# nv-dvl/nerfmatch

Measured on AMD Instinct MI355X. Metric: rays*samples/sec, higher is better.
Workload: dtype fp16x3 (fp16 MFMA on hi/lo-split fp32 operands, three products per fp32 product, fp32 accumulate; fp32 everywhere else)

## Files before the change

nerfmatch_amd/csrc/nerf_fwd_bf16.hip:

```cpp
#include "nerf_split_chain.h"

namespace {
using namespace nmbf;

template <int PART>
__device__ __forceinline__ void tap_prefetch(Ctx& cx) {
  if constexpr (PART == 0) __builtin_amdgcn_s_barrier();
  const char* src = reinterpret_cast<const char*>(cx.tapw);
#pragma unroll
  for (int q = (PART == 0 ? 0 : 4); q < (PART == 0 ? 4 : 7); ++q) {
    const char* sp = src + q * 4096;
    const float* dp = q < 4 ? cx.tap_ring + q * 1024 : cx.tap_ipe + (q - 4) * 1024;
    const unsigned lds = (unsigned)__builtin_amdgcn_readfirstlane((int)(unsigned)(size_t)(const __attribute__((address_space(3))) float*)dp);
    unsigned m0_saved;
    asm volatile("s_mov_b32 %0, m0\n\ts_mov_b32 m0, %1\n\tglobal_load_lds_dwordx4 %2, off\n\tglobal_load_lds_dwordx4 %2, off offset:1024\n\t"
                 "global_load_lds_dwordx4 %2, off offset:2048\n\tglobal_load_lds_dwordx4 %2, off offset:3072\n\ts_mov_b32 m0, %0"
                 : "=&s"(m0_saved) : "s"(lds), "v"(sp) : "memory");
  }
}

__device__ __forceinline__ void dpp_pairs8(float (&o)[8], const float (&x)[8], const float (&y)[8], bool eight) {
  if (eight)
    asm("s_nop 1\n"
        "v_add_f32_dpp %0, %8, %8 row_mirror row_mask:0xf bank_mask:0x3\n\tv_add_f32_dpp %1, %9, %9 row_mirror row_mask:0xf bank_mask:0x3\n\t"
        "v_add_f32_dpp %2, %10, %10 row_mirror row_mask:0xf bank_mask:0x3\n\tv_add_f32_dpp %3, %11, %11 row_mirror row_mask:0xf bank_mask:0x3\n\t"
        "v_add_f32_dpp %4, %12, %12 row_mirror row_mask:0xf bank_mask:0x3\n\tv_add_f32_dpp %5, %13, %13 row_mirror row_mask:0xf bank_mask:0x3\n\t"
        "v_add_f32_dpp %6, %14, %14 row_mirror row_mask:0xf bank_mask:0x3\n\tv_add_f32_dpp %7, %15, %15 row_mirror row_mask:0xf bank_mask:0x3\n\t"
        "v_add_f32_dpp %0, %16, %16 row_mirror row_mask:0xf bank_mask:0xc\n\tv_add_f32_dpp %1, %17, %17 row_mirror row_mask:0xf bank_mask:0xc\n\t"
        "v_add_f32_dpp %2, %18, %18 row_mirror row_mask:0xf bank_mask:0xc\n\tv_add_f32_dpp %3, %19, %19 row_mirror row_mask:0xf bank_mask:0xc\n\t"
        "v_add_f32_dpp %4, %20, %20 row_mirror row_mask:0xf bank_mask:0xc\n\tv_add_f32_dpp %5, %21, %21 row_mirror row_mask:0xf bank_mask:0xc\n\t"
        "v_add_f32_dpp %6, %22, %22 row_mirror row_mask:0xf bank_mask:0xc\n\tv_add_f32_dpp %7, %23, %23 row_mirror row_mask:0xf bank_mask:0xc"
        : "=&v"(o[0]), "=&v"(o[1]), "=&v"(o[2]), "=&v"(o[3]), "=&v"(o[4]), "=&v"(o[5]), "=&v"(o[6]), "=&v"(o[7])
        : "v"(x[0]), "v"(x[1]), "v"(x[2]), "v"(x[3]), "v"(x[4]), "v"(x[5]), "v"(x[6]), "v"(x[7]),
          "v"(y[0]), "v"(y[1]), "v"(y[2]), "v"(y[3]), "v"(y[4]), "v"(y[5]), "v"(y[6]), "v"(y[7]));
  else
    asm("s_nop 1\n"
        "v_add_f32_dpp %0, %8, %8 row_half_mirror row_mask:0xf bank_mask:0x5\n\tv_add_f32_dpp %1, %9, %9 row_half_mirror row_mask:0xf bank_mask:0x5\n\t"
        "v_add_f32_dpp %2, %10, %10 row_half_mirror row_mask:0xf bank_mask:0x5\n\tv_add_f32_dpp %3, %11, %11 row_half_mirror row_mask:0xf bank_mask:0x5\n\t"
        "v_add_f32_dpp %4, %12, %12 row_half_mirror row_mask:0xf bank_mask:0x5\n\tv_add_f32_dpp %5, %13, %13 row_half_mirror row_mask:0xf bank_mask:0x5\n\t"
        "v_add_f32_dpp %6, %14, %14 row_half_mirror row_mask:0xf bank_mask:0x5\n\tv_add_f32_dpp %7, %15, %15 row_half_mirror row_mask:0xf bank_mask:0x5\n\t"
        "v_add_f32_dpp %0, %16, %16 row_half_mirror row_mask:0xf bank_mask:0xa\n\tv_add_f32_dpp %1, %17, %17 row_half_mirror row_mask:0xf bank_mask:0xa\n\t"
        "v_add_f32_dpp %2, %18, %18 row_half_mirror row_mask:0xf bank_mask:0xa\n\tv_add_f32_dpp %3, %19, %19 row_half_mirror row_mask:0xf bank_mask:0xa\n\t"
        "v_add_f32_dpp %4, %20, %20 row_half_mirror row_mask:0xf bank_mask:0xa\n\tv_add_f32_dpp %5, %21, %21 row_half_mirror row_mask:0xf bank_mask:0xa\n\t"
        "v_add_f32_dpp %6, %22, %22 row_half_mirror row_mask:0xf bank_mask:0xa\n\tv_add_f32_dpp %7, %23, %23 row_half_mirror row_mask:0xf bank_mask:0xa"
        : "=&v"(o[0]), "=&v"(o[1]), "=&v"(o[2]), "=&v"(o[3]), "=&v"(o[4]), "=&v"(o[5]), "=&v"(o[6]), "=&v"(o[7])
        : "v"(x[0]), "v"(x[1]), "v"(x[2]), "v"(x[3]), "v"(x[4]), "v"(x[5]), "v"(x[6]), "v"(x[7]),
          "v"(y[0]), "v"(y[1]), "v"(y[2]), "v"(y[3]), "v"(y[4]), "v"(y[5]), "v"(y[6]), "v"(y[7]));
}
template <int XOR>
__device__ __forceinline__ void quad_add8(float (&v)[8]) {
  if (XOR == 1)
    asm("s_nop 1\n"
        "v_add_f32_dpp %0, %0, %0 quad_perm:[1,0,3,2] row_mask:0xf bank_mask:0xf\n\tv_add_f32_dpp %1, %1, %1 quad_perm:[1,0,3,2] row_mask:0xf bank_mask:0xf\n\t"
        "v_add_f32_dpp %2, %2, %2 quad_perm:[1,0,3,2] row_mask:0xf bank_mask:0xf\n\tv_add_f32_dpp %3, %3, %3 quad_perm:[1,0,3,2] row_mask:0xf bank_mask:0xf\n\t"
        "v_add_f32_dpp %4, %4, %4 quad_perm:[1,0,3,2] row_mask:0xf bank_mask:0xf\n\tv_add_f32_dpp %5, %5, %5 quad_perm:[1,0,3,2] row_mask:0xf bank_mask:0xf\n\t"
        "v_add_f32_dpp %6, %6, %6 quad_perm:[1,0,3,2] row_mask:0xf bank_mask:0xf\n\tv_add_f32_dpp %7, %7, %7 quad_perm:[1,0,3,2] row_mask:0xf bank_mask:0xf"
        : "+v"(v[0]), "+v"(v[1]), "+v"(v[2]), "+v"(v[3]), "+v"(v[4]), "+v"(v[5]), "+v"(v[6]), "+v"(v[7]));
  else
    asm("s_nop 1\n"
        "v_add_f32_dpp %0, %0, %0 quad_perm:[2,3,0,1] row_mask:0xf bank_mask:0xf\n\tv_add_f32_dpp %1, %1, %1 quad_perm:[2,3,0,1] row_mask:0xf bank_mask:0xf\n\t"
        "v_add_f32_dpp %2, %2, %2 quad_perm:[2,3,0,1] row_mask:0xf bank_mask:0xf\n\tv_add_f32_dpp %3, %3, %3 quad_perm:[2,3,0,1] row_mask:0xf bank_mask:0xf\n\t"
        "v_add_f32_dpp %4, %4, %4 quad_perm:[2,3,0,1] row_mask:0xf bank_mask:0xf\n\tv_add_f32_dpp %5, %5, %5 quad_perm:[2,3,0,1] row_mask:0xf bank_mask:0xf\n\t"
        "v_add_f32_dpp %6, %6, %6 quad_perm:[2,3,0,1] row_mask:0xf bank_mask:0xf\n\tv_add_f32_dpp %7, %7, %7 quad_perm:[2,3,0,1] row_mask:0xf bank_mask:0xf"
        : "+v"(v[0]), "+v"(v[1]), "+v"(v[2]), "+v"(v[3]), "+v"(v[4]), "+v"(v[5]), "+v"(v[6]), "+v"(v[7]));
}
__device__ __forceinline__ f32x4 reduce_scatter_32rows(float (&v)[128], int lane) {
  float s1[64];
#pragma unroll
  for (int i = 0; i < 64; ++i) {
    const auto r = __builtin_amdgcn_permlane16_swap(__float_as_uint(v[i]), __float_as_uint(v[64 + i]), false, false);
    s1[i] = __uint_as_float(r[0]) + __uint_as_float(r[1]);
  }
  float s2[32];
#pragma unroll
  for (int b = 0; b < 4; ++b) {
    float o[8], x[8], y[8];
#pragma unroll
    for (int i = 0; i < 8; ++i) { x[i] = s1[8 * b + i]; y[i] = s1[32 + 8 * b + i]; }
    dpp_pairs8(o, x, y, true);
#pragma unroll
    for (int i = 0; i < 8; ++i) s2[8 * b + i] = o[i];
  }
  float s3[16];
#pragma unroll
  for (int b = 0; b < 2; ++b) {
    float o[8], x[8], y[8];
#pragma unroll
    for (int i = 0; i < 8; ++i) { x[i] = s2[8 * b + i]; y[i] = s2[16 + 8 * b + i]; }
    dpp_pairs8(o, x, y, false);
#pragma unroll
    for (int i = 0; i < 8; ++i) s3[8 * b + i] = o[i];
  }
  float lo8[8], hi8[8];
#pragma unroll
  for (int i = 0; i < 8; ++i) { lo8[i] = s3[i]; hi8[i] = s3[8 + i]; }
  quad_add8<2>(lo8); quad_add8<2>(hi8);
  float s4[8];
#pragma unroll
  for (int i = 0; i < 8; ++i) s4[i] = (lane & 2) ? hi8[i] : lo8[i];
  float t8[8] = {s4[0], s4[1], s4[2], s4[3], s4[4], s4[5], s4[6], s4[7]};
  quad_add8<1>(t8);
  return (lane & 1) ? f32x4{t8[4], t8[5], t8[6], t8[7]} : f32x4{t8[0], t8[1], t8[2], t8[3]};
}

#define NM_MLP_DONE_WAIT() __builtin_amdgcn_s_waitcnt(0x0070)
#define NM_EPI_BARRIER() asm volatile("s_waitcnt lgkmcnt(0)\n\ts_barrier" ::: "memory")
template <int P>
__device__ __forceinline__ void nerf_fwd_body(const NerfArgs& a) {
  __shared__ __attribute__((aligned(16))) float sm[LDS_TOTAL];
  float* const sm_small = sm + LDS_SMALL;
  float* const ring = sm + LDS_RING;
  float* const sm_ipe = sm + LDS_IPE;
  float* const sm_sigma = sm + LDS_SCR;
  float* const sm_rgb = sm_sigma + TILE;
  float* const sm_t0 = sm_rgb + 3 * TILE;
  float* const sm_t1 = sm_t0 + TILE;
  float* const sm_mean = sm_t1 + TILE;
  float* const sm_dn = sm_mean + 3 * TILE;
  float* const sm_w = sm_dn + TILE;
  float* const sm_misc = sm_w + TILE;
  float* const sm_feat = sm + LDS_FEAT;
  float* const sm_part = sm_feat;
  float* const sm_ex = sm + LDS_EX;
  int* const sm_lray = reinterpret_cast<int*>(sm + LDS_LEFT);
  float* const sm_lT = sm + LDS_LEFT + TILE;
  unsigned* const sm_rng = reinterpret_cast<unsigned*>(sm + LDS_RNG);

  const int tid = threadIdx.x, lane = tid & 63, wave = tid >> 6, s = lane & 31, hi = lane >> 5;
  const bool tail_ok = a.left && !(a.tail_viol && *a.tail_viol != 0);
  const int S = a.S, R = a.R;
  const int Sa = tail_ok ? a.Sa : S;
  const int left = tail_ok ? 1 : 0;
  const int ntiles = tail_ok ? a.ntiles : a.ntiles_full;
  const int SP = Sa < TILE ? Sa : TILE;
  const int nr = TILE / SP;
  const int nchunks = (Sa + TILE - 1) / TILE;
  const bool need_rgb = !(a.flags & NM_NERF_SKIP_RGB);
  const bool feat_max = (a.flags & NM_NERF_FEAT_MAX) != 0;
  const bool need_tap = (a.feat != nullptr) || (a.sfeat != nullptr);
  const int tap = (a.tap < 0 || a.tap > 7) ? 7 : a.tap;
  const int nslots = need_rgb ? NSLOT_FULL : NSLOT_NORGB;
  const char* const blob_slots = a.blob + (size_t)SMALL_PAD * 4;

  for (int i = tid; i < SMALL / 4; i += 256) reinterpret_cast<f32x4*>(sm_small)[i] = reinterpret_cast<const f32x4*>(a.blob)[i];
  if constexpr (P == 2) {
#pragma unroll
    for (int k = 0; k < NRANGE; ++k) sm_rng[k * 256 + tid] = 0u;
  }

  int nleft = 0;
  int bid = blockIdx.x;
#pragma unroll 1
  for (;;) {
  bool lo_pass = false;
  if (left && (nleft > TILE - 4 || (bid >= ntiles && nleft > 0))) lo_pass = true;
  else if (bid >= ntiles) break;
  const int nent = lo_pass ? nleft : 0;
  TRACE(0);
  if (need_rgb && !lo_pass && tid < nr * 48) {
    const int r2 = tid / 48, f = tid % 48;
    const int ray2 = bid * nr + r2;
    const float* rq = a.rays + (size_t)(ray2 < R ? ray2 : R - 1) * 12 + 8;
    float v = 0.f;
    if (f < 24) {
      const int k = (f % 12) / 3;
      const float xe = rq[f % 3] * (float)(1 << k);
      v = nm_sinf(f < 12 ? xe : xe + 1.57079637050628662109375f);
    } else if (f < 27) {
      v = rq[f - 24];
    } else if (f < 43) {
      v = a.app_row ? a.app_row[f - 27] : 0.f;
    }
    if constexpr (P == 2) {
      v *= reinterpret_cast<const float*>(a.blob)[OFF_INSCALE + (f < 27 ? 1 : 2)];
      __hip_atomic_fetch_max(sm_rng + 9 * 256 + tid, __float_as_uint(fabsf(v)), __ATOMIC_RELAXED, __HIP_MEMORY_SCOPE_WORKGROUP);
    }
    sm_ex[tid] = v;
  }
  __syncthreads();
  TRACE(1);

  const int js = wave * 32 + s;
  const int rl = js / SP;
  const int ray = lo_pass ? (js < nent ? sm_lray[js] : R) : bid * nr + rl;
  const int rc = lo_pass ? sm_lray[js < nent ? js : 0] : (ray < R ? ray : R - 1);
  const float* rp = a.rays + (size_t)rc * 12;
  const float o0 = rp[0], o1 = rp[1], o2 = rp[2], d0 = rp[3], d1 = rp[4], d2 = rp[5], radius = rp[11];
  const float dsq0 = d0 * d0, dsq1 = d1 * d1, dsq2 = d2 * d2;
  const float dmag = fmaxf(1e-10f, (dsq0 + dsq1) + dsq2);
  const float dnorm = sqrtf((dsq0 + dsq1) + dsq2);
  const float nul0 = 1.0f - dsq0 / dmag, nul1 = 1.0f - dsq1 / dmag, nul2 = 1.0f - dsq2 / dmag;

  float red_acc = 0.f;
  float carryT = 1.f;
  float best_w = -1.f;
  float feat_run = 0.f;

  const int nch = lo_pass ? 1 : nchunks;
  for (int chunk = 0; chunk < nch; ++chunk) {
    const int sidx = lo_pass ? Sa : chunk * TILE + (js % SP);
    const float t0 = a.t[(size_t)rc * (S + 1) + sidx];
    const float t1 = a.t[(size_t)rc * (S + 1) + sidx + 1];
    const float mu = (t0 + t1) / 2.0f, hw = (t1 - t0) / 2.0f;
    const float mu2 = mu * mu, hw2 = hw * hw, hw4 = hw2 * hw2;
    const float denom = fmaxf(1.1920928955078125e-07f, 3.0f * mu2 + hw2);
    const float t_mean = mu + (2.0f * mu * hw2) / denom;
    const float t_var = hw2 / 3.0f - (float)(4.0 / 15.0) * ((hw4 * (12.0f * mu2 - hw2)) / (denom * denom));
    const float r_var = (radius * radius) * ((mu2 / 4.0f + (float)(5.0 / 12.0) * hw2) - (float)(4.0 / 15.0) * hw4 / denom);
    float mean[3] = {d0 * t_mean + o0, d1 * t_mean + o1, d2 * t_mean + o2};
    float var[3] = {t_var * dsq0 + r_var * nul0, t_var * dsq1 + r_var * nul1, t_var * dsq2 + r_var * nul2};
    if (a.var_scale > 0.f) {
      var[0] *= a.var_scale; var[1] *= a.var_scale; var[2] *= a.var_scale;
    }
    if (hi == 0) {
      sm_t0[js] = t0; sm_t1[js] = t1;
      sm_mean[js] = mean[0]; sm_mean[TILE + js] = mean[1]; sm_mean[2 * TILE + js] = mean[2];
      sm_dn[js] = dnorm;
    }

#pragma unroll
    for (int g0 = 0; g0 < ring_ahead<P>(); ++g0) dma_slot<P>(blob_slots, g0, ring, wave, lane);

    {
      float* dst = sm_ipe + wave * (XS * 2 * 64 * 4) + lane * 4;
      const float ipe_scale = sm_small[OFF_INSCALE];
      const float phl = hi ? 1.57079637050628662109375f : 0.f;
#pragma unroll
      for (int m = 0; m < XS; ++m) {
        float v8[8];
#pragma unroll
        for (int i = 0; i < 8; ++i) {
          const int idx = 8 * m + i;
          const bool live = idx < 45;
          const int ax = (live ? idx : 0) % 3, sb = (live ? idx : 0) / 3;
          const float mu = mean[ax], vr = var[ax];
          const float sc = (float)(1 << sb);
          const float xe = mu * sc;
          float v = __builtin_amdgcn_exp2f((-0.5f * (vr * (sc * sc))) * 1.44269504088896340736f) * sin32(xe + phl);
          if constexpr (P == 2) v *= ipe_scale;
          v8[i] = live ? v : 0.f;
        }
        if constexpr (is_split<P>()) {
          bf16x8 h8, l8;
          split8_p<P>(v8, h8, l8);
          *reinterpret_cast<u32x4*>(dst + (m * 2 + 0) * 256) = __builtin_bit_cast(u32x4, h8);
          *reinterpret_cast<u32x4*>(dst + (m * 2 + 1) * 256) = __builtin_bit_cast(u32x4, l8);
        } else {
          *reinterpret_cast<u32x4*>(dst + m * 256) = __builtin_bit_cast(u32x4, pack8_f16(v8));
        }
      }
    }

    TRACE(2);
    Ctx cx;
    cx.blob_slots = blob_slots; cx.ring = ring; cx.sm_small = sm_small;
    cx.tapw = reinterpret_cast<f32x4*>(a.ws) + ((size_t)blockIdx.x * 4 + wave) * 32 * 64 + lane;
    cx.nslots = nslots; cx.wave = wave; cx.lane = lane; cx.hi = hi; cx.tap = need_tap ? tap : -1; cx.g = 0; cx.sig_part = 0.f;
    cx.vmax = 0.f; cx.rng = sm_rng + tid; cx.sc = 1.f;
    cx.tap_pref = need_tap && !lo_pass; cx.rgb = need_rgb;
    cx.tap_ring = ring + wave * SLOT_FLOATS; cx.tap_ipe = sm_ipe + wave * (XS * 2 * 64 * 4);
    if constexpr (is_split<P>()) {
      NM_WAIT_VMCNT(8);
      __builtin_amdgcn_s_barrier();
    } else {
      ring_acquire<P>(blob_slots, 0, nslots, ring, wave, lane);
    }
    load_half<P>(cx.opA, ring, lane, 0);
    if constexpr (P == 1) load_half<1>(cx.opB, ring, lane, 1);
    const float* ipe_src = sm_ipe + wave * (XS * 2 * 64 * 4) + lane * 4;
    f32x16 acc[8];
    ipe_steps<P, true>(acc, cx, ipe_src);
    finish_layer<P>(acc, 0, cx);
    TRACE(3);
#pragma unroll 1
    for (int l = 1; l < 8; ++l) {
      layer_pass<P>(acc, l, cx, ipe_src);
      TRACE(3 + l);
    }
    float c_r = 0.f, c_g = 0.f, c_b = 0.f;
    if (!need_rgb) {
      if (cx.tap == 7) dump_tap(7, cx);
      NM_MLP_DONE_WAIT();
      if (cx.tap_pref) tap_prefetch<0>(cx);
      alpha_head(cx);
      if (cx.tap_pref) tap_prefetch<1>(cx);
    } else {
      const int hh = launder(lane) >> 5;
      const float* exr = sm_ex + launder(rl) * 48 + 8 * hh;
      f32x16 av[4];
      views_hidden<P>(av, cx);
      fold_range<P>(cx, 7);
      bf16x8 exh[VS], exl[VS];
#pragma unroll
      for (int e = 0; e < VS; ++e) {
        float v8[8];
        if (!lo_pass) {
          const f32x4 e0 = *reinterpret_cast<const f32x4*>(exr + 16 * e), e1 = *reinterpret_cast<const f32x4*>(exr + 16 * e + 4);
          v8[0] = e0[0]; v8[1] = e0[1]; v8[2] = e0[2]; v8[3] = e0[3]; v8[4] = e1[0]; v8[5] = e1[1]; v8[6] = e1[2]; v8[7] = e1[3];
        } else {
          const float* rq = a.rays + (size_t)launder(rc) * 12 + 8;
          const float vd0 = rq[0], vd1 = rq[1], vd2 = rq[2];
#pragma unroll
          for (int i = 0; i < 8; ++i) {
            const int f = 16 * e + 8 * hh + i;
            const int ax = f % 3;
            const float dax = ax == 0 ? vd0 : ax == 1 ? vd1 : vd2;
            float v = 0.f;
            if (f < 24) {
              const float xe = dax * (float)(1 << ((f % 12) / 3));
              v = nm_sinf(f < 12 ? xe : xe + 1.57079637050628662109375f);
            } else if (f < 27) {
              v = dax;
            } else if (f < 43) {
              v = a.app_row ? a.app_row[f - 27] : 0.f;
            }
            if constexpr (P == 2) v *= sm_small[OFF_INSCALE + (f < 27 ? 1 : 2)];
            v8[i] = v;
          }
        }
        if constexpr (is_split<P>()) split8_p<P>(v8, exh[e], exl[e]);
        else exh[e] = exl[e] = pack8_f16(v8);
      }
      views_extras<P>(av, cx, exh, exl);
      TRACE(11);
      NM_MLP_DONE_WAIT();
      if (cx.tap_pref) tap_prefetch<0>(cx);
      const float* bv = sm_small + OFF_BVIEWS + 4 * hh;
      const float* wr = sm_small + OFF_WRGB + 4 * hh;
      float pr = 0.f, pg = 0.f, pb = 0.f;
#pragma unroll
      for (int ob = 0; ob < 4; ++ob) {
#pragma unroll
        for (int q = 0; q < 4; ++q) {
          const f32x4 b4 = *reinterpret_cast<const f32x4*>(bv + ob * 32 + 8 * q);
          const f32x4 wr4 = *reinterpret_cast<const f32x4*>(wr + ob * 32 + 8 * q);
          const f32x4 wg4 = *reinterpret_cast<const f32x4*>(wr + 128 + ob * 32 + 8 * q);
          const f32x4 wb4 = *reinterpret_cast<const f32x4*>(wr + 256 + ob * 32 + 8 * q);
#pragma unroll
          for (int e = 0; e < 4; ++e) {
            const float hv = __builtin_fmaxf(acc_read(av[ob][4 * q + e]) + b4[e], 0.f);
            pr = NM_FMA(hv, wr4[e], pr);
            pg = NM_FMA(hv, wg4[e], pg);
            pb = NM_FMA(hv, wb4[e], pb);
          }
        }
      }
      pr = (pr + nm_shfl_xor32(pr)) + sm_small[OFF_MISC + 1];
      pg = (pg + nm_shfl_xor32(pg)) + sm_small[OFF_MISC + 2];
      pb = (pb + nm_shfl_xor32(pb)) + sm_small[OFF_MISC + 3];
      c_r = 1.0f / (1.0f + expf(-pr));
      c_g = 1.0f / (1.0f + expf(-pg));
      c_b = 1.0f / (1.0f + expf(-pb));
      if (cx.tap_pref) tap_prefetch<1>(cx);
    }
    const float sigma_raw = (cx.sig_part + nm_shfl_xor32(cx.sig_part)) + sm_small[OFF_MISC];
    TRACE(12);
    {
      const int jsw = launder(js);
      if ((launder(lane) >> 5) == 0) {
        sm_sigma[jsw] = sigma_raw;
        sm_rgb[jsw] = c_r; sm_rgb[TILE + jsw] = c_g; sm_rgb[2 * TILE + jsw] = c_b;
      }
    }
    NM_EPI_BARRIER();
    TRACE(13);
    const int tid2 = launder(threadIdx.x), lane2 = tid2 & 63, wave2 = tid2 >> 6;

    if (lo_pass) {
      if (tid2 < nent) {
        const int ray2 = sm_lray[tid2];
        const float sg = fmaxf(sm_sigma[tid2], 0.f);
        const float delta = (sm_t1[tid2] - sm_t0[tid2]) * sm_dn[tid2];
        const float wgt = (1.0f - expf(-sg * delta)) * sm_lT[tid2];
        sm_w[tid2] = wgt;
        a.weights[(size_t)ray2 * S + Sa] = wgt;
        if (a.acc) atomicAdd(a.acc + ray2, wgt);
        if (a.rgb && need_rgb) {
#pragma unroll
          for (int c = 0; c < 3; ++c) atomicAdd(a.rgb + (size_t)ray2 * 3 + c, a.white_bg ? wgt * sm_rgb[c * TILE + tid2] - wgt : wgt * sm_rgb[c * TILE + tid2]);
        }
        if (a.depth) atomicAdd(a.depth + ray2, wgt * (0.5f * (sm_t0[tid2] + sm_t1[tid2])));
        if (a.pts) {
#pragma unroll
          for (int c = 0; c < 3; ++c) atomicAdd(a.pts + (size_t)ray2 * 3 + c, wgt * sm_mean[c * TILE + tid2]);
        }
      }
      __syncthreads();
      if (need_tap) {
        const int jl = launder(js), hl = launder(lane) >> 5;
        const f32x4* tw = reinterpret_cast<const f32x4*>(a.ws) + ((size_t)blockIdx.x * 4 + wave2) * 32 * 64 + lane2;
        if (jl < nent) {
          const int ray2 = sm_lray[jl];
          const float desc = sm_small[OFF_DESCALE + tap];
          const float wj = sm_w[jl] * desc;
#pragma unroll 4
          for (int ks = 0; ks < HS; ++ks) {
            const f32x4 ta = tw[(2 * ks) * 64], tb = tw[(2 * ks + 1) * 64];
            const int n0 = (ks >> 1) * 32 + 16 * (ks & 1) + 4 * hl;
            if (a.sfeat) {
              float* dsf = a.sfeat + ((size_t)ray2 * S + Sa) * 256 + n0;
              *reinterpret_cast<f32x4*>(dsf) = ta * desc;
              *reinterpret_cast<f32x4*>(dsf + 8) = tb * desc;
            }
            if (a.feat) {
              float* df = a.feat + (size_t)ray2 * 256 + n0;
#pragma unroll
              for (int e = 0; e < 4; ++e) {
                atomicAdd(df + e, wj * ta[e]);
                atomicAdd(df + 8 + e, wj * tb[e]);
              }
            }
          }
        }
      }
      __syncthreads();
      break;
    }

    float alpha = 0.f, incl = 1.f;
    if (tid2 < TILE) {
      const float sg = fmaxf(sm_sigma[tid2], 0.f);
      const float delta = (sm_t1[tid2] - sm_t0[tid2]) * sm_dn[tid2];
      alpha = 1.0f - expf(-sg * delta);
      incl = (1.0f - alpha) + 1e-10f;
      const int seg = SP < 64 ? SP : 64;
#pragma unroll
      for (int dlt = 1; dlt < 64; dlt <<= 1) {
        const float up = __shfl_up(incl, dlt, 64);
        if (dlt < seg && (lane2 & (seg - 1)) >= dlt) incl *= up;
      }
      if (lane2 == 63) sm_misc[wave2] = incl;
    }
    NM_EPI_BARRIER();
    if (tid2 < TILE) {
      const int seg = SP < 64 ? SP : 64;
      float excl = __shfl_up(incl, 1, 64);
      if ((lane2 & (seg - 1)) == 0) excl = 1.f;
      if (SP == TILE && wave2 == 1) excl *= sm_misc[0];
      excl *= carryT;
      const float wgt = alpha * excl;
      sm_w[tid2] = wgt;
      const int r2 = tid2 / SP, ray2 = bid * nr + r2;
      if (ray2 < R) {
        const int s2 = chunk * TILE + tid2 % SP;
        a.weights[(size_t)ray2 * S + s2] = wgt;
        if (left && chunk == nchunks - 1) {
          for (int k = Sa + 1 + tid2 % SP; k < S; k += SP) a.weights[(size_t)ray2 * S + k] = 0.f;
          if (tid2 % SP == SP - 1) {
            sm_lray[nleft + r2] = ray2;
            sm_lT[nleft + r2] = excl * ((1.0f - alpha) + 1e-10f);
          }
        }
        if (a.raw && !NM_TRACE) {
          f32x4 rv = {sm_rgb[tid2], sm_rgb[TILE + tid2], sm_rgb[2 * TILE + tid2], sm_sigma[tid2]};
          *reinterpret_cast<f32x4*>(a.raw + ((size_t)ray2 * S + s2) * 4) = rv;
        }
      }
      float pq[8] = {wgt, wgt * sm_rgb[tid2], wgt * sm_rgb[TILE + tid2], wgt * sm_rgb[2 * TILE + tid2],
                     wgt * (0.5f * (sm_t0[tid2] + sm_t1[tid2])), wgt * sm_mean[tid2], wgt * sm_mean[TILE + tid2],
                     wgt * sm_mean[2 * TILE + tid2]};
      nm_half_sum_dpp8(pq);
      if ((tid2 & 31) == 16) {
        *reinterpret_cast<f32x4*>(sm_part + (tid2 >> 5) * 8) = f32x4{pq[0], pq[1], pq[2], pq[3]};
        *reinterpret_cast<f32x4*>(sm_part + (tid2 >> 5) * 8 + 4) = f32x4{pq[4], pq[5], pq[6], pq[7]};
      }
    }
    if (nchunks > 1) carryT = carryT * (sm_misc[0] * sm_misc[1]);
    NM_EPI_BARRIER();

    if (tid2 < 8 * nr) {
      const int q = tid2 & 7, r2 = tid2 >> 3;
      const float* wv = sm_w + r2 * SP;
      if (!feat_max || q < 5) {
        float sum = 0.f;
        for (int hw = r2 * (SP / 32); hw < (r2 + 1) * (SP / 32); ++hw) sum += sm_part[hw * 8 + q];
        red_acc += sum;
      }
      if (feat_max) {
        float bw = wv[0];
        int bi = 0;
        for (int k = 1; k < SP; ++k)
          if (wv[k] > bw) { bw = wv[k]; bi = k; }
        const bool better = bw > best_w;
        if (better) best_w = bw;
        if (q == 0) sm_misc[8 + r2] = better ? __int_as_float(r2 * SP + bi) : __int_as_float(-1);
        if (q >= 5 && better) red_acc = sm_mean[(q - 5) * TILE + r2 * SP + bi];
      }
    }
    if (feat_max) NM_EPI_BARRIER();

    TRACE(14);
    if (need_tap) {
      const int jl = launder(js), hl = launder(lane) >> 5;
      f32x4 tapv[2 * HS];
      {
        asm volatile("s_waitcnt vmcnt(0)" ::: "memory");
        f32x4 tail[4];
        {
          const f32x4* tw = reinterpret_cast<const f32x4*>(a.ws) + ((size_t)blockIdx.x * 4 + (launder(threadIdx.x) >> 6)) * 32 * 64 + (launder(threadIdx.x) & 63);
#pragma unroll
          for (int i = 0; i < 4; ++i) tail[i] = tw[(28 + i) * 64];
        }
        const float* lr = ring + (launder(threadIdx.x) >> 6) * SLOT_FLOATS + (launder(threadIdx.x) & 63) * 4;
        const float* li = sm_ipe + (launder(threadIdx.x) >> 6) * (XS * 2 * 64 * 4) + (launder(threadIdx.x) & 63) * 4;
#pragma unroll
        for (int c = 0; c < 2 * HS; ++c)
          tapv[c] = c < 16 ? *reinterpret_cast<const f32x4*>(lr + c * 256) : c < 28 ? *reinterpret_cast<const f32x4*>(li + (c - 16) * 256) : tail[c - 28];
      }
      const float desc = sm_small[OFF_DESCALE + tap];
      const float wj = sm_w[jl] * desc;
      const int rsel = jl / SP;
      const int best = feat_max ? __float_as_int(sm_misc[8 + rsel]) : -2;
      float* prow = sm_feat + (jl >> 5) * 256 + 4 * hl;
      if (a.sfeat && ray < R) {
#pragma unroll
        for (int ks = 0; ks < HS; ++ks) {
          const f32x4 ta = tapv[2 * ks], tb = tapv[2 * ks + 1];
          float* dsf = a.sfeat + ((size_t)ray * S + sidx) * 256 + (ks >> 1) * 32 + 16 * (ks & 1) + 4 * hl;
          *reinterpret_cast<f32x4*>(dsf) = ta * desc;
          *reinterpret_cast<f32x4*>(dsf + 8) = tb * desc;
        }
      }
      if (a.feat) {
        float wv[128];
        const float mult = feat_max ? (jl == best ? desc : 0.f) : wj;
#pragma unroll
        for (int c = 0; c < 2 * HS; ++c)
#pragma unroll
          for (int e = 0; e < 4; ++e) wv[4 * c + e] = mult * tapv[c][e];
        const f32x4 sum4 = reduce_scatter_32rows(wv, jl);
        const int r = jl & 31;
        *reinterpret_cast<f32x4*>(prow + (r >> 2) * 32 + 16 * ((r >> 1) & 1) + 8 * (r & 1)) = sum4;
      }
    }
    TRACE(15);
    __syncthreads();
    TRACE(16);
    if (a.feat) {
      const int wpr = SP / 32;
      for (int r2 = 0; r2 < nr; ++r2) {
        float f = 0.f;
        bool any = !feat_max;
        if (feat_max) {
          const int best = __float_as_int(sm_misc[8 + r2]);
          any = best >= 0;
        }
        for (int w2 = 0; w2 < wpr; ++w2) f += sm_feat[(r2 * wpr + w2) * 256 + tid2];
        const int ray2 = bid * nr + r2;
        if (nchunks > 1) {
          if (feat_max) { if (any) feat_run = f; }
          else feat_run += f;
          f = feat_run;
        }
        if (ray2 < R && chunk == nchunks - 1 && (any || nchunks > 1)) a.feat[(size_t)ray2 * 256 + tid2] = f;
      }
    }
    __syncthreads();
  }

  if (lo_pass) {
    nleft = 0;
    continue;
  }
  if (tid < 8 * nr) {
    const int q = tid & 7, r2 = tid >> 3, ray2 = bid * nr + r2;
    const float accv = __shfl(red_acc, lane & ~7, 64);
    if (ray2 < R) {
      if (q == 0) { if (a.acc) a.acc[ray2] = red_acc; }
      else if (q <= 3) { if (a.rgb && need_rgb) a.rgb[(size_t)ray2 * 3 + (q - 1)] = a.white_bg ? red_acc + (1.0f - accv) : red_acc; }
      else if (q == 4) { if (a.depth) a.depth[ray2] = red_acc; }
      else { if (a.pts) a.pts[(size_t)ray2 * 3 + (q - 5)] = red_acc; }
    }
  }
  TRACE(17);
  if (left) nleft += (R - bid * nr) < nr ? (R - bid * nr) : nr;
  bid += gridDim.x;
  }
  if constexpr (P == 2) {
    __syncthreads();
    if (a.status && tid < NRANGE) {
      unsigned m = 0u;
      for (int i = 0; i < 256; ++i) m = max(m, sm_rng[tid * 256 + ((i + 32 * tid) & 255)]);
      if (m) atomicMax(reinterpret_cast<unsigned*>(a.status) + 1 + tid, m);
      if (m >= __float_as_uint(F16_MAX)) atomicOr(a.status, 1);
    }
  }
}

__global__ void __launch_bounds__(256, 1) nerf_fwd_bf16x3_kernel(NerfArgs a) { nerf_fwd_body<0>(a); }
__global__ void __launch_bounds__(256, 1) nerf_fwd_fp16x1_kernel(NerfArgs a) { nerf_fwd_body<1>(a); }
__global__ void __launch_bounds__(256, 1) nerf_fwd_fp16x3_kernel(NerfArgs a) { nerf_fwd_body<2>(a); }

}

extern "C" size_t nm_nerf_workspace_bytes_bf16x3(void) { return (size_t)WS_WORKGROUPS * TILE * 256 * sizeof(float); }

static int nerf_fwd_split(int mode, const void* blob, const float* rays, const float* t, const float* app_row, int R, int S, int tap_layer,
                          int white_bg, float var_scale, int flags, float* weights, float* feat, float* pts, float* rgb, float* depth,
                          float* acc, float* raw, float* sample_feat, void* workspace, const int* zero_tail_violation, nmStream_t stream,
                          int* status = nullptr) {
  NM_CHECK_ARG(blob && rays && t && weights && R > 0 && S > 0);
  if (!(S == 32 || S == 64 || (S % 128) == 0)) return NM_ERR_UNSUPPORTED;
  if (tap_layer > 7) return NM_ERR_ARG;
  if ((feat || sample_feat) && !workspace) return NM_ERR_WORKSPACE;
  NerfArgs a;
  a.ws = (float*)workspace;
  a.blob = (const char*)blob; a.rays = rays; a.t = t; a.app_row = app_row;
  a.weights = weights; a.feat = feat; a.pts = pts; a.rgb = rgb; a.depth = depth; a.acc = acc; a.raw = raw; a.sfeat = sample_feat;
  a.R = R; a.S = S; a.tap = tap_layer; a.white_bg = white_bg; a.flags = flags; a.var_scale = var_scale;
  a.status = status;
  const bool zero_tail = (flags & NM_NERF_ZERO_TAIL) && (S == 64 || S == 128 || (S >= 256 && S % 256 == 0)) && !raw && !sample_feat &&
                         !(flags & NM_NERF_FEAT_MAX);
  a.Sa = zero_tail ? S / 2 : S;
  a.left = zero_tail ? 1 : 0;
  const int SP = a.Sa < TILE ? a.Sa : TILE, nr = TILE / SP;
  a.ntiles = (R + nr - 1) / nr;
  const int SPf = S < TILE ? S : TILE, nrf = TILE / SPf;
  a.ntiles_full = (R + nrf - 1) / nrf;
  a.tail_viol = zero_tail ? zero_tail_violation : nullptr;
  const int ncu = nm_stream_cus(stream);
  const int grid = a.ntiles < ncu ? a.ntiles : (ncu < WS_WORKGROUPS ? ncu : WS_WORKGROUPS);
  if (mode == 1) nerf_fwd_fp16x1_kernel<<<grid, 256, 0, (hipStream_t)stream>>>(a);
  else if (mode == 2) nerf_fwd_fp16x3_kernel<<<grid, 256, 0, (hipStream_t)stream>>>(a);
  else nerf_fwd_bf16x3_kernel<<<grid, 256, 0, (hipStream_t)stream>>>(a);
  return nm_launch_status();
}

extern "C" int nm_nerf_fwd_bf16x3(const void* blob, const float* rays, const float* t, const float* app_row, int R, int S,
                                  int tap_layer, int white_bg, float var_scale, int flags, float* weights, float* feat, float* pts,
                                  float* rgb, float* depth, float* acc, float* raw, float* sample_feat, void* workspace,
                                  const int* zero_tail_violation, nmStream_t stream) {
  return nerf_fwd_split(0, blob, rays, t, app_row, R, S, tap_layer, white_bg, var_scale, flags, weights, feat, pts, rgb, depth, acc, raw,
                        sample_feat, workspace, zero_tail_violation, stream);
}

extern "C" int nm_nerf_fwd_fp16x1(const void* blob, const float* rays, const float* t, const float* app_row, int R, int S,
                                  int tap_layer, int white_bg, float var_scale, int flags, float* weights, float* feat, float* pts,
                                  float* rgb, float* depth, float* acc, float* raw, float* sample_feat, void* workspace,
                                  const int* zero_tail_violation, nmStream_t stream) {
  return nerf_fwd_split(1, blob, rays, t, app_row, R, S, tap_layer, white_bg, var_scale, flags, weights, feat, pts, rgb, depth, acc, raw,
                        sample_feat, workspace, zero_tail_violation, stream);
}

extern "C" int nm_nerf_fwd_fp16x3(const void* blob, const float* rays, const float* t, const float* app_row, int R, int S,
                                  int tap_layer, int white_bg, float var_scale, int flags, float* weights, float* feat, float* pts,
// ... 6 lines not shown
```

nerfmatch_amd/csrc/nerf_split_chain.h:

```cpp
#pragma once
#include "nerf_bf16_common.h"

namespace nmbf {

template <int P> constexpr bool is_bf16() { return P == 0 || P == 4; }
template <int P> constexpr bool has_gates() { return P == 4; }
typedef _Float16 f16x8 __attribute__((ext_vector_type(8)));
typedef _Float16 f16x2 __attribute__((ext_vector_type(2)));
template <int P>
__device__ __forceinline__ f32x16 mfma_p(const bf16x8& a, const bf16x8& b, const f32x16& c) {
  if constexpr (is_bf16<P>()) return MFMA_BF16(a, b, c);
  else return __builtin_amdgcn_mfma_f32_32x32x16_f16(__builtin_bit_cast(f16x8, a), __builtin_bit_cast(f16x8, b), c, 0, 0, 0);
}
template <int P> constexpr bool is_split() { return P != 1; }
template <int P> constexpr int slot_bytes() { return is_split<P>() ? SLOT_BYTES : SLOT_BYTES / 2; }
template <int P> constexpr int slot_floats() { return slot_bytes<P>() / 4; }
template <int P> constexpr int ring_slots() { return is_split<P>() ? NRING : 2 * NRING; }
template <int P> constexpr int ring_ahead() { return is_split<P>() ? 4 : 6; }
constexpr float F16_MAX = 65504.0f;
__device__ __forceinline__ void split8_f16(const float (&v)[8], bf16x8& hi, bf16x8& lo) {
  f16x8 h8, l8;
#pragma unroll
  for (int i = 0; i < 8; ++i) {
    const float c = __builtin_amdgcn_fmed3f(v[i], -F16_MAX, F16_MAX);
// ... 388 lines not shown
  const int g = cx.g;
  const OpHalf C = cx.opA;
  work.prefetch();
  if constexpr (!EVEN) ring_acquire_two<P>(cx.blob_slots, g, cx.ring, cx.wave, cx.lane);
#pragma unroll
  for (int o = 0; o < 4; ++o) {
    acc[o] = mfma_p<P>(C.h[o], xh, FIRST ? zero : acc[o]);
    __builtin_amdgcn_sched_barrier(0);
    work(o);
    __builtin_amdgcn_sched_barrier(0);
  }
  load_half<P>(cx.opA, cx.ring + ((g + 1) & (NRING - 1)) * SLOT_FLOATS, cx.lane, 0);
  __builtin_amdgcn_sched_barrier(0);
#pragma unroll
  for (int o = 0; o < 4; ++o) {
    acc[o] = mfma_p<P>(C.h[o], xl, acc[o]);
    __builtin_amdgcn_sched_barrier(0);
    work(4 + o);
    __builtin_amdgcn_sched_barrier(0);
  }
#pragma unroll
  for (int o = 0; o < 4; ++o) {
    acc[o] = mfma_p<P>(C.l[o], xh, acc[o]);
    __builtin_amdgcn_sched_barrier(0);
    work(8 + o);
    __builtin_amdgcn_sched_barrier(0);
  }
  cx.g = g + 1;
}

template <int P, bool FIRST, bool EVEN, class W0, class W1>
__device__ __forceinline__ void slot_step4x2(f32x16 (&av)[4], Ctx& cx, const bf16x8& x0h, const bf16x8& x0l, Unit& u1, W0 w0, W1 w1) {
  const f32x16 zero = {0.f, 0.f, 0.f, 0.f, 0.f, 0.f, 0.f, 0.f, 0.f, 0.f, 0.f, 0.f, 0.f, 0.f, 0.f, 0.f};
  const int g = cx.g;
  const OpHalf A = cx.opA;
  OpHalf B;
  w0.prefetch();
#pragma unroll
  for (int o = 0; o < 4; ++o) {
    av[o] = mfma_p<P>(A.h[o], x0h, FIRST ? zero : av[o]);
    __builtin_amdgcn_sched_barrier(0);
    w0(o);
    __builtin_amdgcn_sched_barrier(0);
  }
  load_half<P>(B, cx.ring + (g & (NRING - 1)) * SLOT_FLOATS, cx.lane, 1);
  __builtin_amdgcn_sched_barrier(0);
#pragma unroll
  for (int o = 0; o < 4; ++o) {
    av[o] = mfma_p<P>(A.h[o], x0l, av[o]);
    __builtin_amdgcn_sched_barrier(0);
    w0(4 + o);
    __builtin_amdgcn_sched_barrier(0);
  }
#pragma unroll
  for (int o = 0; o < 4; ++o) {
    av[o] = mfma_p<P>(A.l[o], x0h, av[o]);
    __builtin_amdgcn_sched_barrier(0);
    w0(8 + o);
    __builtin_amdgcn_sched_barrier(0);
  }
  if constexpr (!EVEN) ring_acquire_two<P>(cx.blob_slots, g, cx.ring, cx.wave, cx.lane);
  const bf16x8 x1h = __builtin_bit_cast(bf16x8, u1.h), x1l = __builtin_bit_cast(bf16x8, u1.l);
  w1.prefetch();
#pragma unroll
  for (int o = 0; o < 4; ++o) {
    av[o] = mfma_p<P>(B.h[o], x1h, av[o]);
    __builtin_amdgcn_sched_barrier(0);
    w1(o);
    __builtin_amdgcn_sched_barrier(0);
  }
  load_half<P>(cx.opA, cx.ring + ((g + 1) & (NRING - 1)) * SLOT_FLOATS, cx.lane, 0);
  __builtin_amdgcn_sched_barrier(0);
#pragma unroll
  for (int o = 0; o < 4; ++o) {
    av[o] = mfma_p<P>(B.h[o], x1l, av[o]);
    __builtin_amdgcn_sched_barrier(0);
    w1(4 + o);
    __builtin_amdgcn_sched_barrier(0);
  }
#pragma unroll
  for (int o = 0; o < 4; ++o) {
    av[o] = mfma_p<P>(B.l[o], x1h, av[o]);
    __builtin_amdgcn_sched_barrier(0);
    w1(8 + o);
    __builtin_amdgcn_sched_barrier(0);
  }
  cx.g = g + 1;
}

template <int P>
__device__ __forceinline__ void views_hidden(f32x16 (&av)[4], Ctx& cx) {
  if constexpr (is_split<P>()) {
#pragma unroll
    for (int sl = 0; sl < HS / 2; ++sl) {
      const Unit x0 = cx.xn;
      Unit u1;
      const bf16x8 x0h = __builtin_bit_cast(bf16x8, x0.h), x0l = __builtin_bit_cast(bf16x8, x0.l);
      if (sl == 0) slot_step4x2<P, true, true>(av, cx, x0h, x0l, u1, unit_work<P>(1, 7, cx, u1), unit_work<P>(2, 7, cx, cx.xn));
      else if (sl + 1 == HS / 2) slot_step4x2<P, false, false>(av, cx, x0h, x0l, u1, unit_work<P>(2 * sl + 1, 7, cx, u1), NoWork{});
      else if (sl & 1) slot_step4x2<P, false, false>(av, cx, x0h, x0l, u1, unit_work<P>(2 * sl + 1, 7, cx, u1), unit_work<P>(2 * sl + 2, 7, cx, cx.xn));
      else slot_step4x2<P, false, true>(av, cx, x0h, x0l, u1, unit_work<P>(2 * sl + 1, 7, cx, u1), unit_work<P>(2 * sl + 2, 7, cx, cx.xn));
    }
  } else {
#pragma unroll
    for (int ks = 0; ks < HS; ks += 2) {
      {
        const Unit xc = cx.xn;
        if (ks == 0) slot_step4<P, true, true>(av, cx, __builtin_bit_cast(bf16x8, xc.h), __builtin_bit_cast(bf16x8, xc.l), unit_work<P>(ks + 1, 7, cx, cx.xn));
        else slot_step4<P, false, true>(av, cx, __builtin_bit_cast(bf16x8, xc.h), __builtin_bit_cast(bf16x8, xc.l), unit_work<P>(ks + 1, 7, cx, cx.xn));
      }
      {
        const Unit xc = cx.xn;
        if (ks + 2 < HS) slot_step4<P, false, false>(av, cx, __builtin_bit_cast(bf16x8, xc.h), __builtin_bit_cast(bf16x8, xc.l), unit_work<P>(ks + 2, 7, cx, cx.xn));
        else slot_step4<P, false, false>(av, cx, __builtin_bit_cast(bf16x8, xc.h), __builtin_bit_cast(bf16x8, xc.l), NoWork{});
      }
    }
  }
}
template <int P>
__device__ __forceinline__ void views_extras(f32x16 (&av)[4], Ctx& cx, const bf16x8 (&eh)[VS], const bf16x8 (&el)[VS]) {
  if constexpr (is_split<P>()) {
    Unit u1;
    u1.h = __builtin_bit_cast(u32x4, eh[1]); u1.l = __builtin_bit_cast(u32x4, el[1]);
    slot_step4x2<P, false, true>(av, cx, eh[0], el[0], u1, NoWork{}, NoWork{});
    slot_step4<P, false, false>(av, cx, eh[2], el[2], NoWork{});
  } else {
#pragma unroll
    for (int e = 0; e < VS; ++e) {
      if (e & 1) slot_step4<P, false, false>(av, cx, eh[e], el[e], NoWork{});
      else slot_step4<P, false, true>(av, cx, eh[e], el[e], NoWork{});
    }
  }
}

template <int P, bool FIRST>
__device__ __forceinline__ void ipe_steps(f32x16 (&acc)[8], Ctx& cx, const float* ipe_src) {
  auto operand = [&](int m, bf16x8& ph, bf16x8& pl) {
    ph = __builtin_bit_cast(bf16x8, *reinterpret_cast<const u32x4*>(ipe_src + (is_split<P>() ? (m * 2 + 0) : m) * 256));
    pl = ph;
    if constexpr (is_split<P>()) pl = __builtin_bit_cast(bf16x8, *reinterpret_cast<const u32x4*>(ipe_src + (m * 2 + 1) * 256));
  };
#pragma unroll
  for (int m = 0; m < XS; m += 2) {
    bf16x8 ph, pl;
    operand(m, ph, pl);
    if (m == 0) slot_step8<P, FIRST, true>(acc, cx, ph, pl, NoWork{});
    else slot_step8<P, false, true>(acc, cx, ph, pl, NoWork{});
    operand(m + 1, ph, pl);
    if (m + 2 == XS) slot_step8<P, false, false>(acc, cx, ph, pl, AccTake<P>{acc, cx});
    else slot_step8<P, false, false>(acc, cx, ph, pl, NoWork{});
  }
}

template <int P>
__device__ __forceinline__ void layer_pass(f32x16 (&acc)[8], int l, Ctx& cx, const float* ipe_src) {
  if (l - 1 == cx.tap) dump_tap(l - 1, cx);
#pragma unroll
  for (int ks = 0; ks < HS; ks += 2) {
    {
      const Unit xc = cx.xn;
      if (ks == 0) slot_step8<P, true, true>(acc, cx, __builtin_bit_cast(bf16x8, xc.h), __builtin_bit_cast(bf16x8, xc.l), unit_work<P>(ks + 1, l - 1, cx, cx.xn));
      else slot_step8<P, false, true>(acc, cx, __builtin_bit_cast(bf16x8, xc.h), __builtin_bit_cast(bf16x8, xc.l), unit_work<P>(ks + 1, l - 1, cx, cx.xn));
    }
    {
      const Unit xc = cx.xn;
      if (ks + 2 < HS) slot_step8<P, false, false>(acc, cx, __builtin_bit_cast(bf16x8, xc.h), __builtin_bit_cast(bf16x8, xc.l), unit_work<P>(ks + 2, l - 1, cx, cx.xn));
      else slot_step8<P, false, false>(acc, cx, __builtin_bit_cast(bf16x8, xc.h), __builtin_bit_cast(bf16x8, xc.l), AccTake<P>{acc, cx});
    }
  }
  fold_range<P>(cx, l - 1);
  if constexpr (has_gates<P>()) {
    cx.gptr[(l - 1) * 256] = u32x4{cx.gbits[0], cx.gbits[1], cx.gbits[2], cx.gbits[3]};
    cx.gbits[0] = cx.gbits[1] = cx.gbits[2] = cx.gbits[3] = 0u;
  }
  if (l == 5) ipe_steps<P, false>(acc, cx, ipe_src);
  finish_layer<P>(acc, l, cx);
  if (l == 7) {
    if (cx.rgb) {
      if (cx.tap == 7) dump_tap(7, cx);
      alpha_head(cx);
    }
  }
}

}
```

Measured before the change: 363.3 million.

## Reduce tap-7 features from registers right after alpha head, skipping workspace dump

When the feature tap is layer 7 and only dense features are requested, the kernel now computes compositing weights right after the alpha head. It then reduces the layer-7 activations, weighted per sample, directly from registers through permlane/DPP reductions into the feature LDS rows. This skips writing the tap to the global workspace and re-reading it in the epilogue. The compositing code is split into reusable lambdas, and sm_part is moved to sm_misc scratch so it no longer aliases sm_feat. In exchange the tap-7 activations must stay live in registers longer, and extra barriers are added inside the layer loop.

```diff
diff --git a/nerfmatch_amd/csrc/nerf_fwd_bf16.hip b/nerfmatch_amd/csrc/nerf_fwd_bf16.hip
--- a/nerfmatch_amd/csrc/nerf_fwd_bf16.hip
+++ b/nerfmatch_amd/csrc/nerf_fwd_bf16.hip
@@ -64,13 +64,11 @@
         "v_add_f32_dpp %6, %6, %6 quad_perm:[2,3,0,1] row_mask:0xf bank_mask:0xf\n\tv_add_f32_dpp %7, %7, %7 quad_perm:[2,3,0,1] row_mask:0xf bank_mask:0xf"
         : "+v"(v[0]), "+v"(v[1]), "+v"(v[2]), "+v"(v[3]), "+v"(v[4]), "+v"(v[5]), "+v"(v[6]), "+v"(v[7]));
 }
-__device__ __forceinline__ f32x4 reduce_scatter_32rows(float (&v)[128], int lane) {
-  float s1[64];
-#pragma unroll
-  for (int i = 0; i < 64; ++i) {
-    const auto r = __builtin_amdgcn_permlane16_swap(__float_as_uint(v[i]), __float_as_uint(v[64 + i]), false, false);
-    s1[i] = __uint_as_float(r[0]) + __uint_as_float(r[1]);
-  }
+__device__ __forceinline__ float reduce_scatter_step16(float x, float y) {
+  const auto r = __builtin_amdgcn_permlane16_swap(__float_as_uint(x), __float_as_uint(y), false, false);
+  return __uint_as_float(r[0]) + __uint_as_float(r[1]);
+}
+__device__ __forceinline__ f32x4 reduce_scatter_16pairs(const float (&s1)[64], int lane) {
   float s2[32];
 #pragma unroll
   for (int b = 0; b < 4; ++b) {
@@ -101,6 +99,12 @@
   float t8[8] = {s4[0], s4[1], s4[2], s4[3], s4[4], s4[5], s4[6], s4[7]};
   quad_add8<1>(t8);
   return (lane & 1) ? f32x4{t8[4], t8[5], t8[6], t8[7]} : f32x4{t8[0], t8[1], t8[2], t8[3]};
+}
+__device__ __forceinline__ f32x4 reduce_scatter_32rows(float (&v)[128], int lane) {
+  float s1[64];
+#pragma unroll
+  for (int i = 0; i < 64; ++i) s1[i] = reduce_scatter_step16(v[i], v[64 + i]);
+  return reduce_scatter_16pairs(s1, lane);
 }
 
 #define NM_MLP_DONE_WAIT() __builtin_amdgcn_s_waitcnt(0x0070)
@@ -119,8 +123,8 @@
   float* const sm_dn = sm_mean + 3 * TILE;
   float* const sm_w = sm_dn + TILE;
   float* const sm_misc = sm_w + TILE;
+  float* const sm_part = sm_misc + 32;
   float* const sm_feat = sm + LDS_FEAT;
-  float* const sm_part = sm_feat;
   float* const sm_ex = sm + LDS_EX;
   int* const sm_lray = reinterpret_cast<int*>(sm + LDS_LEFT);
   float* const sm_lT = sm + LDS_LEFT + TILE;
@@ -257,7 +261,8 @@
     cx.tapw = reinterpret_cast<f32x4*>(a.ws) + ((size_t)blockIdx.x * 4 + wave) * 32 * 64 + lane;
     cx.nslots = nslots; cx.wave = wave; cx.lane = lane; cx.hi = hi; cx.tap = need_tap ? tap : -1; cx.g = 0; cx.sig_part = 0.f;
     cx.vmax = 0.f; cx.rng = sm_rng + tid; cx.sc = 1.f;
-    cx.tap_pref = need_tap && !lo_pass; cx.rgb = need_rgb;
+    const bool early = need_rgb && !lo_pass && tap == 7 && a.feat && !a.sfeat;
+    cx.tap_pref = need_tap && !lo_pass && !early; cx.rgb = need_rgb;
     cx.tap_ring = ring + wave * SLOT_FLOATS; cx.tap_ipe = sm_ipe + wave * (XS * 2 * 64 * 4);
     if constexpr (is_split<P>()) {
       NM_WAIT_VMCNT(8);
@@ -268,13 +273,122 @@
     load_half<P>(cx.opA, ring, lane, 0);
     if constexpr (P == 1) load_half<1>(cx.opB, ring, lane, 1);
     const float* ipe_src = sm_ipe + wave * (XS * 2 * 64 * 4) + lane * 4;
+
+    auto composite_weights = [&]() __attribute__((always_inline)) {
+      const int tid2 = launder(threadIdx.x), lane2 = tid2 & 63, wave2 = tid2 >> 6;
+      float alpha = 0.f, incl = 1.f;
+      if (tid2 < TILE) {
+        const float sg = fmaxf(sm_sigma[tid2], 0.f);
+        const float delta = (sm_t1[tid2] - sm_t0[tid2]) * sm_dn[tid2];
+        alpha = 1.0f - expf(-sg * delta);
+        incl = (1.0f - alpha) + 1e-10f;
+        const int seg = SP < 64 ? SP : 64;
+#pragma unroll
+        for (int dlt = 1; dlt < 64; dlt <<= 1) {
+          const float up = __shfl_up(incl, dlt, 64);
+          if (dlt < seg && (lane2 & (seg - 1)) >= dlt) incl *= up;
+        }
+        if (lane2 == 63) sm_misc[wave2] = incl;
+      }
+      NM_EPI_BARRIER();
+      if (tid2 < TILE) {
+        const int seg = SP < 64 ? SP : 64;
+        float excl = __shfl_up(incl, 1, 64);
+        if ((lane2 & (seg - 1)) == 0) excl = 1.f;
+        if (SP == TILE && wave2 == 1) excl *= sm_misc[0];
+        excl *= carryT;
+        sm_w[tid2] = alpha * excl;
+        const int r2 = tid2 / SP, ray2 = bid * nr + r2;
+        if (left && chunk == nchunks - 1 && ray2 < R && tid2 % SP == SP - 1) {
+          sm_lray[nleft + r2] = ray2;
+          sm_lT[nleft + r2] = excl * ((1.0f - alpha) + 1e-10f);
+        }
+      }
+      if (nchunks > 1) carryT = carryT * (sm_misc[0] * sm_misc[1]);
+    };
+    auto composite_sums = [&]() __attribute__((always_inline)) {
+      const int tid2 = launder(threadIdx.x);
+      if (tid2 < TILE) {
+        const float wgt = sm_w[tid2];
+        const int r2 = tid2 / SP, ray2 = bid * nr + r2;
+        if (ray2 < R) {
+          const int s2 = chunk * TILE + tid2 % SP;
+          a.weights[(size_t)ray2 * S + s2] = wgt;
+          if (left && chunk == nchunks - 1) {
+            for (int k = Sa + 1 + tid2 % SP; k < S; k += SP) a.weights[(size_t)ray2 * S + k] = 0.f;
+          }
+          if (a.raw && !NM_TRACE) {
+            f32x4 rv = {sm_rgb[tid2], sm_rgb[TILE + tid2], sm_rgb[2 * TILE + tid2], sm_sigma[tid2]};
+            *reinterpret_cast<f32x4*>(a.raw + ((size_t)ray2 * S + s2) * 4) = rv;
+          }
+        }
+        float pq[8] = {wgt, wgt * sm_rgb[tid2], wgt * sm_rgb[TILE + tid2], wgt * sm_rgb[2 * TILE + tid2],
+                       wgt * (0.5f * (sm_t0[tid2] + sm_t1[tid2])), wgt * sm_mean[tid2], wgt * sm_mean[TILE + tid2],
+                       wgt * sm_mean[2 * TILE + tid2]};
+        nm_half_sum_dpp8(pq);
+        if ((tid2 & 31) == 16) {
+          *reinterpret_cast<f32x4*>(sm_part + (tid2 >> 5) * 8) = f32x4{pq[0], pq[1], pq[2], pq[3]};
+          *reinterpret_cast<f32x4*>(sm_part + (tid2 >> 5) * 8 + 4) = f32x4{pq[4], pq[5], pq[6], pq[7]};
+        }
+      }
+    };
+    auto pick_best = [&]() __attribute__((always_inline)) {
+      const int tid2 = launder(threadIdx.x);
+      if (tid2 < 8 * nr) {
+        const int q = tid2 & 7, r2 = tid2 >> 3;
+        const float* wv = sm_w + r2 * SP;
+        float bw = wv[0];
+        int bi = 0;
+        for (int k = 1; k < SP; ++k)
+          if (wv[k] > bw) { bw = wv[k]; bi = k; }
+        const bool better = bw > best_w;
+        if (better) best_w = bw;
+        if (q == 0) sm_misc[8 + r2] = better ? __int_as_float(r2 * SP + bi) : __int_as_float(-1);
+        if (q >= 5 && better) red_acc = sm_mean[(q - 5) * TILE + r2 * SP + bi];
+      }
+    };
+    auto tap7_early = [&](Ctx& c) __attribute__((always_inline)) {
+      const int t2 = launder(threadIdx.x), jl = (t2 >> 6) * 32 + (t2 & 31), hl = (t2 >> 5) & 1;
+      const float sigma_raw = (c.sig_part + nm_shfl_xor32(c.sig_part)) + sm_small[OFF_MISC];
+      if (hl == 0) sm_sigma[jl] = sigma_raw;
+      NM_EPI_BARRIER();
+      composite_weights();
+      NM_EPI_BARRIER();
+      if (feat_max) {
+        pick_best();
+        NM_EPI_BARRIER();
+      }
+      const float desc = sm_small[OFF_DESCALE + 7];
+      const float wj = sm_w[jl] * desc;
+      const int best = feat_max ? __float_as_int(sm_misc[8 + jl / SP]) : -2;
+      const float mult = feat_max ? (jl == best ? desc : 0.f) : wj;
+      const float* bl = sm_small + OFF_BIAS + 7 * 256 + 4 * hl;
+      const float s7 = sm_small[OFF_SCALE + 7];
+      float s1[64];
+#pragma unroll
+      for (int cq = 0; cq < HS; ++cq) {
+        const f32x4 b0 = *reinterpret_cast<const f32x4*>(bl + (cq >> 2) * 32 + 8 * (cq & 3));
+        const f32x4 b1 = *reinterpret_cast<const f32x4*>(bl + (4 + (cq >> 2)) * 32 + 8 * (cq & 3));
+#pragma unroll
+        for (int e = 0; e < 4; ++e) {
+          const float x = mult * __builtin_fmaxf(__builtin_fmaf(c.hv[4 * cq + e], s7, b0[e]), 0.f);
+          const float y = mult * __builtin_fmaxf(__builtin_fmaf(c.hv[64 + 4 * cq + e], s7, b1[e]), 0.f);
+          s1[4 * cq + e] = reduce_scatter_step16(x, y);
+        }
+      }
+      const f32x4 sum4 = reduce_scatter_16pairs(s1, jl);
+      const int r = jl & 31;
+      float* prow = sm_feat + (jl >> 5) * 256 + 4 * hl;
+      *reinterpret_cast<f32x4*>(prow + (r >> 2) * 32 + 16 * ((r >> 1) & 1) + 8 * (r & 1)) = sum4;
+    };
+    const Tap7InRegisters<decltype(tap7_early)> tap7{early, tap7_early};
     f32x16 acc[8];
     ipe_steps<P, true>(acc, cx, ipe_src);
     finish_layer<P>(acc, 0, cx);
     TRACE(3);
 #pragma unroll 1
     for (int l = 1; l < 8; ++l) {
-      layer_pass<P>(acc, l, cx, ipe_src);
+      layer_pass<P>(acc, l, cx, ipe_src, tap7);
       TRACE(3 + l);
     }
     float c_r = 0.f, c_g = 0.f, c_b = 0.f;
@@ -417,80 +531,25 @@
       break;
     }
 
-    float alpha = 0.f, incl = 1.f;
-    if (tid2 < TILE) {
-      const float sg = fmaxf(sm_sigma[tid2], 0.f);
-      const float delta = (sm_t1[tid2] - sm_t0[tid2]) * sm_dn[tid2];
-      alpha = 1.0f - expf(-sg * delta);
-      incl = (1.0f - alpha) + 1e-10f;
-      const int seg = SP < 64 ? SP : 64;
-#pragma unroll
-      for (int dlt = 1; dlt < 64; dlt <<= 1) {
-        const float up = __shfl_up(incl, dlt, 64);
-        if (dlt < seg && (lane2 & (seg - 1)) >= dlt) incl *= up;
-      }
-      if (lane2 == 63) sm_misc[wave2] = incl;
-    }
-    NM_EPI_BARRIER();
-    if (tid2 < TILE) {
-      const int seg = SP < 64 ? SP : 64;
-      float excl = __shfl_up(incl, 1, 64);
-      if ((lane2 & (seg - 1)) == 0) excl = 1.f;
-      if (SP == TILE && wave2 == 1) excl *= sm_misc[0];
-      excl *= carryT;
-      const float wgt = alpha * excl;
-      sm_w[tid2] = wgt;
-      const int r2 = tid2 / SP, ray2 = bid * nr + r2;
-      if (ray2 < R) {
-        const int s2 = chunk * TILE + tid2 % SP;
-        a.weights[(size_t)ray2 * S + s2] = wgt;
-        if (left && chunk == nchunks - 1) {
-          for (int k = Sa + 1 + tid2 % SP; k < S; k += SP) a.weights[(size_t)ray2 * S + k] = 0.f;
-          if (tid2 % SP == SP - 1) {
-            sm_lray[nleft + r2] = ray2;
-            sm_lT[nleft + r2] = excl * ((1.0f - alpha) + 1e-10f);
-          }
-        }
-        if (a.raw && !NM_TRACE) {
-          f32x4 rv = {sm_rgb[tid2], sm_rgb[TILE + tid2], sm_rgb[2 * TILE + tid2], sm_sigma[tid2]};
-          *reinterpret_cast<f32x4*>(a.raw + ((size_t)ray2 * S + s2) * 4) = rv;
-        }
-      }
-      float pq[8] = {wgt, wgt * sm_rgb[tid2], wgt * sm_rgb[TILE + tid2], wgt * sm_rgb[2 * TILE + tid2],
-                     wgt * (0.5f * (sm_t0[tid2] + sm_t1[tid2])), wgt * sm_mean[tid2], wgt * sm_mean[TILE + tid2],
-                     wgt * sm_mean[2 * TILE + tid2]};
-      nm_half_sum_dpp8(pq);
-      if ((tid2 & 31) == 16) {
-        *reinterpret_cast<f32x4*>(sm_part + (tid2 >> 5) * 8) = f32x4{pq[0], pq[1], pq[2], pq[3]};
-        *reinterpret_cast<f32x4*>(sm_part + (tid2 >> 5) * 8 + 4) = f32x4{pq[4], pq[5], pq[6], pq[7]};
-      }
-    }
-    if (nchunks > 1) carryT = carryT * (sm_misc[0] * sm_misc[1]);
+    if (!early) composite_weights();
+    composite_sums();
     NM_EPI_BARRIER();
 
     if (tid2 < 8 * nr) {
       const int q = tid2 & 7, r2 = tid2 >> 3;
-      const float* wv = sm_w + r2 * SP;
       if (!feat_max || q < 5) {
         float sum = 0.f;
         for (int hw = r2 * (SP / 32); hw < (r2 + 1) * (SP / 32); ++hw) sum += sm_part[hw * 8 + q];
         red_acc += sum;
       }
-      if (feat_max) {
-        float bw = wv[0];
-        int bi = 0;
-        for (int k = 1; k < SP; ++k)
-          if (wv[k] > bw) { bw = wv[k]; bi = k; }
-        const bool better = bw > best_w;
-        if (better) best_w = bw;
-        if (q == 0) sm_misc[8 + r2] = better ? __int_as_float(r2 * SP + bi) : __int_as_float(-1);
-        if (q >= 5 && better) red_acc = sm_mean[(q - 5) * TILE + r2 * SP + bi];
-      }
-    }
-    if (feat_max) NM_EPI_BARRIER();
+    }
+    if (feat_max && !early) {
+      pick_best();
+      NM_EPI_BARRIER();
+    }
 
     TRACE(14);
-    if (need_tap) {
+    if (need_tap && !early) {
       const int jl = launder(js), hl = launder(lane) >> 5;
       f32x4 tapv[2 * HS];
       {
diff --git a/nerfmatch_amd/csrc/nerf_split_chain.h b/nerfmatch_amd/csrc/nerf_split_chain.h
--- a/nerfmatch_amd/csrc/nerf_split_chain.h
+++ b/nerfmatch_amd/csrc/nerf_split_chain.h
@@ -564,8 +564,18 @@
   }
 }
 
-template <int P>
-__device__ __forceinline__ void layer_pass(f32x16 (&acc)[8], int l, Ctx& cx, const float* ipe_src) {
+struct Tap7Workspace {
+  static constexpr bool on = false;
+  __device__ __forceinline__ void fn(Ctx&) const {}
+};
+template <class F>
+struct Tap7InRegisters {
+  bool on;
+  F fn;
+};
+
+template <int P, class Tap7 = Tap7Workspace>
+__device__ __forceinline__ void layer_pass(f32x16 (&acc)[8], int l, Ctx& cx, const float* ipe_src, const Tap7& tap7 = Tap7()) {
   if (l - 1 == cx.tap) dump_tap(l - 1, cx);
 #pragma unroll
   for (int ks = 0; ks < HS; ks += 2) {
@@ -589,10 +599,11 @@
   finish_layer<P>(acc, l, cx);
   if (l == 7) {
     if (cx.rgb) {
-      if (cx.tap == 7) dump_tap(7, cx);
+      if (cx.tap == 7 && !tap7.on) dump_tap(7, cx);
       alpha_head(cx);
-    }
-  }
-}
-
-}
+      if (tap7.on) tap7.fn(cx);
+    }
+  }
+}
+
+}
```

After: 376.4 million, median of 6. 3.6% higher.
